# iit-DLSLab/gym-quadruped

Measured on AMD Instinct MI355X. Metric: env-steps/sec (batched), higher is better.
Workload: dtype f32; 1 GPU; mini_cheetah flat, 4096 envs/GPU, random-action rollout (50*N(0,1) torques), ALL_OBS (227 scalars), auto-reset on termination (next_step), sim_dt 0.002, newton solver <=100 it tol 1e-8, robot self-collision on (mesh pairs: GJK / EPA on the hulls, as mjc_Convex); envs_per_gpu=4096, total_envs=4096, parallelism=env-shards x1 (no collectives)

## Files before the change

### gym_quadruped_amd/csrc/gq_boxes.h

```cpp
#pragma once
#include "gq_step_kernel.h"
#include "gq_pairs.h"
#include "gq_convex.h"
#include "gq_exchange.h"

namespace gq {

#define GQ_BX_WCLS(W) (reinterpret_cast<int32_t*>(&(W).F[0][32]))
#define GQ_BX_LGNRM(W) (&(W).F[1][0])
#define GQ_BX_CONNRM(W) (&(W).F[1][3 * GQ_MAXLG])
#define GQ_BX_ISPH(W) (&(W).u.B[40][0])
#define GQ_BX_OBBW 13
#define GQ_BX_OBB(W) (&(W).u.B[0][0])
#define GQ_CVX_SHP(W) ((LdsF)&(W).F[0][44])
#define GQ_CVX_POLY_BOX(W) ((LdsF)&(W).u.B[28][0])
#define GQ_CVX_POLY_SELF(W) ((LdsF)&(W).u.B[38][0])
static_assert(GQ_BX_OBBW * GQ_MAXLG <= 28 * GQ_NVD && 28 * GQ_NVD + GQ_CVX_POLY_WORDS <= 40 * GQ_NVD && 38 * GQ_NVD + GQ_CVX_POLY_WORDS <= 64 * GQ_NVD && 44 + GQ_CVX_SHP_WORDS <= GQ_FACTOR_SIZE,
              "scratch of the convex routine");

__device__ __forceinline__ float sphere_box(V3 c, V3 s, float r, V3& n) {
  const V3 q = v3(med3(c.x, -s.x, s.x), med3(c.y, -s.y, s.y), med3(c.z, -s.z, s.z));
  const V3 d = c - q;
  const float l2 = dot(d, d);
  if (l2 > 0.0f) {
// ... 530 lines not shown
  } else {
    const int tot = bcast(wave_incl_scan(nfit | ((nfit * need) << 8) | ((nfit * vres) << 18)), 63);
    const int found = bcast(incl_all, 63) & 0xff;
    ncon += tot & 0xff;
    rows += (tot >> 8) & 0x3ff;
    if constexpr (CONE) reserve += (tot >> 18) & 0x3ff;
    S.ndrop += found - (tot & 0xff);
  }
}

__device__ __forceinline__ void closest_seg_seg(V3 p1, V3 q1, V3 p2, V3 q2, V3& c1, V3& c2) {
  const V3 d1 = q1 - p1, d2 = q2 - p2, r = p1 - p2;
  const float a = dot(d1, d1), e = dot(d2, d2), f = dot(d2, r), EPS = 1e-12f;
  float s, t;
  if (a <= EPS && e <= EPS) { s = 0.0f; t = 0.0f; }
  else if (a <= EPS) { s = 0.0f; t = med3(fdiv(f, e), 0.0f, 1.0f); }
  else {
    const float c = dot(d1, r);
    if (e <= EPS) { t = 0.0f; s = med3(fdiv(-c, a), 0.0f, 1.0f); }
    else {
      const float b = dot(d1, d2), den = a * e - b * b;
      s = den > 1e-6f * a * e ? med3(fdiv(b * f - c * e, den), 0.0f, 1.0f) : 0.0f;
      const float ie = fast_rcp(e), ia = fast_rcp(a);
      t = (b * s + f) * ie;
      if (t < 0.0f) { t = 0.0f; s = med3(-c * ia, 0.0f, 1.0f); }
      else if (t > 1.0f) { t = 1.0f; s = med3((b - c) * ia, 0.0f, 1.0f); }
    }
  }
  c1 = p1 + s * d1; c2 = p2 + t * d2;
}

#define GQ_CON_BODY2(x) ((x) & 0xff)
#define GQ_CON_BODY1(x) (((x) >> 8) - 1)
#define GQ_WCLS_SELF (-2)

struct SelfPrefetch { float caps[7], bsph[4]; int32_t body, it1[2], it2[2], bp[2]; };
__device__ __forceinline__ SelfPrefetch self_prefetch(const GQ_MODEL GqDevModel& m, const int nlg, const int nsp) {
  const int lane = lane_id();
  SelfPrefetch P;
  const int it = lane < 4 + nlg ? lane : 0;
#pragma unroll
  for (int i = 0; i < 7; i++) P.caps[i] = m.item_caps[it][i];
#pragma unroll
  for (int i = 0; i < 4; i++) P.bsph[i] = m.item_bsph[it][i];
  P.body = m.item_body[it];
#pragma unroll
  for (int h = 0; h < 2; h++) {
    const int p = h * GQ_WAVE + lane < nsp ? h * GQ_WAVE + lane : 0;
    P.it1[h] = m.sp[p].it1; P.it2[h] = m.sp[p].it2; P.bp[h] = m.sp[p].bp;
  }
  return P;
}

__device__ inline void self_item_shape(const WaveMem& W, const GQ_MODEL GqDevModel& m, const int it, const float* k, LdsF dst) {
  CvxShape S;
  const int pt = it < 4 ? 2 : m.lg[it - 4].ptype;
  if (pt == 2 || pt == 3) {
    S.kind = 2; S.adr = 0; S.num = 2; S.pm = -1; S.t = ld3(k); S.h = ld3(k + 3); S.r = k[6];
#pragma unroll
    for (int i = 0; i < 9; i++) S.R[i] = (i % 4 == 0) ? 1.0f : 0.0f;
  } else {
    const GQ_MODEL GqDevGeom& G = m.lg[it - 4];
    const float* Rb = W.xmat[G.body];
    S.kind = 0; S.adr = G.plane_adr; S.num = G.cloud_num; S.pm = G.cap_adr; S.r = G.radius; S.h = v3(0.0f, 0.0f, 0.0f);
#pragma unroll
    for (int i = 0; i < 3; i++)
#pragma unroll
      for (int j = 0; j < 3; j++) S.R[3 * i + j] = Rb[3 * i] * G.mat[j] + Rb[3 * i + 1] * G.mat[3 + j] + Rb[3 * i + 2] * G.mat[6 + j];
    S.t = ld3(W.xpos[G.body]) + matvec(Rb, ld3(G.pos));
  }
  cvx_shape_store(dst, S);
}
__device__ inline void self_item_obb(const WaveMem& W, const GQ_MODEL GqDevModel& m, const int it, const float* k, V3& c, float* R, V3& h) {
  const int pt = it < 4 ? 2 : m.lg[it - 4].ptype;
  if (pt == 2 || pt == 3) {
    const V3 p0 = ld3(k), p1 = ld3(k + 3);
    c = 0.5f * (p0 + p1);
    h = v3(0.5f * fabsf(p1.x - p0.x) + k[6], 0.5f * fabsf(p1.y - p0.y) + k[6], 0.5f * fabsf(p1.z - p0.z) + k[6]);
#pragma unroll
    for (int i = 0; i < 9; i++) R[i] = (i % 4 == 0) ? 1.0f : 0.0f;
  } else {
    const GQ_MODEL GqDevGeom& G = m.lg[it - 4];
    const float* Rb = W.xmat[G.body];
#pragma unroll
    for (int i = 0; i < 3; i++)
#pragma unroll
      for (int j = 0; j < 3; j++) R[3 * i + j] = Rb[3 * i] * G.mat[j] + Rb[3 * i + 1] * G.mat[3 + j] + Rb[3 * i + 2] * G.mat[6 + j];
    c = ld3(W.xpos[G.body]) + matvec(Rb, ld3(G.pos)) + matvec(R, ld3(G.aabb_c));
    h = v3(G.aabb_h[0] + G.radius, G.aabb_h[1] + G.radius, G.aabb_h[2] + G.radius);
  }
}

#define GQ_COLD_HINT(c) (COLD ? __builtin_expect((long)(c), 0L) : (long)(c))

__device__ inline void sepc_store(const WaveMem& W, float* row, V3 d) {
  const float dd = dot(d, d);
  V3 b = v3(0.0f, 0.0f, 0.0f);
  if (dd > 1e-24f) b = fast_rsqrt(dd) * matTvec(W.xmat[0], d);
  row[0] = b.x; row[1] = b.y; row[2] = b.z;
}

__device__ inline bool self_hulls_apart(const WaveMem& W, const GQ_MODEL GqDevModel& m, const GQ_MODEL float* vx, int it1, const float* k1, const float* R1,
                                        int it2, const float* k2, const float* R2, float marg, bool use_dir = false, V3 dir = {0.0f, 0.0f, 0.0f}) {
  V3 t[2]; float r[2]; int adr[2]; bool seg[2];
#pragma unroll
  for (int s = 0; s < 2; s++) {
    const int it = s ? it2 : it1; const float* k = s ? k2 : k1;
    const int pt = it < 4 ? 2 : m.lg[it - 4].ptype;
    seg[s] = pt == 2 || pt == 3;
    if (seg[s]) { t[s] = 0.5f * (ld3(k) + ld3(k + 3)); r[s] = k[6]; adr[s] = -1; }
    else { const GQ_MODEL GqDevGeom& G = m.lg[it - 4]; t[s] = ld3(W.xpos[G.body]) + matvec(W.xmat[G.body], ld3(G.pos)); r[s] = G.radius; adr[s] = G.hgrid_adr; if (adr[s] < 0) return false; }
  }
  const V3 d = use_dir ? dir : t[1] - t[0];
  const float dd = dot(d, d);
  if (!(dd > 1e-12f)) return false;
  const float hA = seg[0] ? fmaxf(dot(ld3(k1), d), dot(ld3(k1 + 3), d)) : dot(t[0], d) + cvx_hgrid(vx, adr[0], matTvec(R1, d));
  const float hB = seg[1] ? fmaxf(-dot(ld3(k2), d), -dot(ld3(k2 + 3), d)) : -dot(t[1], d) + cvx_hgrid(vx, adr[1], matTvec(R2, -1.0f * d));
  return -hA - hB > (marg + r[0] + r[1] + 1e-5f) * fast_sqrt(dd);
}

template <bool CONE, bool PRIM = true, bool COLD = false, bool CVX = true>
__device__ inline void append_self_contacts(WaveMem& W, const GQ_MODEL GqDevModel& m, float mu_env, WorldAppend& S, const SelfPrefetch& pre, const StepConsts& K, const int nlg, const GQ_MODEL GqDevBatch& Bt, float* xdbg = nullptr, const int env = 0) {
  constexpr int NP = PRIM ? 4 : 1;
  const int lane = lane_id();
  const int nsp = K.nsp;
  if (nsp == 0) return;
  int32_t* xq_tab = nullptr; int xq_slots = 0;
  float* sepc = nullptr;
  int xq_pre = 0;
  (void)Bt; (void)env; (void)xdbg;
  if constexpr (CVX) {
#ifndef GQ_XQ_OFF
    xq_tab = Bt.xq; xq_slots = Bt.xq_slots;
#endif
    sepc = Bt.sepc ? Bt.sepc + (size_t)env * Bt.sepc_stride : nullptr;
    if (xq_tab) { Xq X0; X0.q = xq_tab; X0.slots = xq_slots; xq_pre = ld_pub(xq_tab + xq_window(X0, wave_index()) + lane); }
  }
  const uint64_t lt = lane == 0 ? 0ull : (~0ull >> (64 - lane));
  float(*cw)[12] = reinterpret_cast<float(*)[12]>(&W.u.B[0][0]);
  {
    const int it = lane < 4 + nlg ? lane : 0;
    const int b = pre.body;
    const V3 o = ld3(W.xpos[b]);
    const V3 e0 = o + matvec(W.xmat[b], v3(pre.caps[0], pre.caps[1], pre.caps[2])), e1 = o + matvec(W.xmat[b], v3(pre.caps[3], pre.caps[4], pre.caps[5]));
    st3(cw[it], e0); st3(cw[it] + 3, e1);
    cw[it][6] = pre.caps[6];
    st3(cw[it] + 8, o + matvec(W.xmat[b], v3(pre.bsph[0], pre.bsph[1], pre.bsph[2])));
    cw[it][11] = pre.bsph[3];
  }
  uint64_t near[2] = {~0ull, ~0ull};
  if (nsp > 2 * GQ_WAVE) {
#pragma unroll
    for (int half = 0; half < 2; half++) {
      const int p = half * GQ_WAVE + lane;
      bool nr = false;
      if (p < m.nbp) {
        const GQ_MODEL GqDevBodyPair& P = m.bp[p];
        const V3 d = ld3(W.xpos[P.b2]) + matvec(W.xmat[P.b2], ld3(m.body_sph[P.b2])) - ld3(W.xpos[P.b1]) - matvec(W.xmat[P.b1], ld3(m.body_sph[P.b1]));
        const float rr = m.body_sph[P.b1][3] + m.body_sph[P.b2][3] + K.self_margin;
        nr = dot(d, d) < rr * rr;
      }
      near[half] = ballot(nr);
    }
  }
  uint64_t live_pass = ~0ull;
  if constexpr (CONE) if (nsp > 2 * GQ_WAVE) {
    const int np = (nsp + GQ_WAVE - 1) / GQ_WAVE, lp = lane < np ? lane : 0;
    const uint64_t pb0 = m.sp_pass_bp[lp][0], pb1 = m.sp_pass_bp[lp][1];
    live_pass = ballot(lane < np && ((near[0] & pb0) | (near[1] & pb1)) != 0);
  }
  if (K.self_cut == 1) { wave_barrier(); return; }
  wave_barrier();
  GQ_SUB(W, 1, 10);
  int32_t* list = reinterpret_cast<int32_t*>(&W.u.B[30][0]);
  int ncand = 0;
#pragma unroll 1
  for (int p0 = 0; p0 < nsp; p0 += GQ_WAVE) {
    if constexpr (CONE) if (!((live_pass >> (p0 / GQ_WAVE)) & 1ull)) continue;
    const int p = p0 + lane;
    bool cand;
    {
      int it1, it2, bp;
      if (p0 == 0) { it1 = pre.it1[0]; it2 = pre.it2[0]; bp = pre.bp[0]; }
      else if (p0 == GQ_WAVE) { it1 = pre.it1[1]; it2 = pre.it2[1]; bp = pre.bp[1]; }
      else { const GQ_MODEL GqDevSelfPair& P = m.sp[p < nsp ? p : 0]; it1 = P.it1; it2 = P.it2; bp = P.bp; }
      const bool nr = (near[(bp >> 6) & 1] >> (bp & 63)) & 1;
      const float* k1 = cw[it1] + 8;
      const float* k2 = cw[it2] + 8;
      const V3 dm = ld3(k2) - ld3(k1);
      const float reach = k1[3] + k2[3] + K.self_margin;
      cand = p < nsp && nr && dot(dm, dm) < reach * reach;
    }
    const uint64_t cm = ballot(cand);
    if (cm == 0) continue;
    const int at = ncand + popc64(cm & lt);
    if (cand && at < 2 * GQ_WAVE) list[at] = p;
    ncand += popc64(cm);
  }
  GQ_SUB(W, 1, 11);
  int xq_act = 0, xq_hlp = 0;
  if constexpr (CVX) { xq_act = bcast(xq_pre, 31); xq_hlp = bcast(xq_pre, 63); }
  if (K.self_cut == 2) return;
  if (ncand == 0) {
    if constexpr (!CVX) return;
    else {
      if (xq_tab == nullptr) return;
      Xq X0; X0.q = xq_tab; X0.slots = xq_slots;
      xq_mark_helper(X0, wave_index(), xq_hlp);
      if (!xq_is_hot(xq_act, wall_clock64())) return;
    }
  }
  if (ncand > 2 * GQ_WAVE) ncand = 2 * GQ_WAVE;
  wave_barrier();
  const int npass = ncand > 0 ? ncand : 1;
#pragma unroll 1
  for (int c0 = 0; c0 < npass; c0 += GQ_WAVE) {
    const bool cand = c0 + lane < ncand;
    const int p = cand ? list[c0 + lane] : 0;
    PairHit H;
    H.n = 0;
    int it1 = 0, it2 = 0;
    bool cvx = false;
    if (cand) {
      const GQ_MODEL GqDevSelfPair& Pp = m.sp[p];
      it1 = Pp.it1; it2 = Pp.it2;
      const int kind = Pp.kind;
      const float marg = Pp.mix.margin;
      const float* k1 = cw[it1];
      const float* k2 = cw[it2];
      if (kind == 0) {
        V3 c1, c2;
        closest_seg_seg(ld3(k1), ld3(k1 + 3), ld3(k2), ld3(k2 + 3), c1, c2);
        const V3 d = c2 - c1;
        const float l2 = dot(d, d), len = fast_sqrt(l2), dist = len - k1[6] - k2[6];
        if (dist < marg && len >= 1e-9f) {
          const V3 nrm = fast_rcp(len) * d;
          H.n = 1; H.dist[0] = dist; H.nrm[0] = nrm; H.pos[0] = c1 + (k1[6] + 0.5f * dist) * nrm;
        }
      } else if (kind == 4) { if constexpr (CVX) {
        V3 c1, h1, c2, h2; float R1[9], R2[9];
        self_item_obb(W, m, it1, k1, c1, R1, h1);
        self_item_obb(W, m, it2, k2, c2, R2, h2);
        cvx = !obb_apart(c1, R1, h1, c2, R2, h2, marg);
        if (cvx) cvx = !self_hulls_apart(W, m, K.vx, it1, k1, R1, it2, k2, R2, marg);
        if (cvx && sepc) {
          const float* c = sepc + 3 * Pp.cidx;
          const V3 dw = matvec(W.xmat[0], v3(c[0], c[1], c[2]));
          if (dot(dw, dw) > 0.25f) cvx = !self_hulls_apart(W, m, K.vx, it1, k1, R1, it2, k2, R2, marg, true, dw);
        }
      } } else if constexpr (PRIM) {
        const int ib = kind == 2 ? it2 : it1;
        bool continue_pair = true;
        const GQ_MODEL GqDevGeom& G = m.lg[ib - 4];
        const float* Rb = W.xmat[G.body];
        float A[9];
#pragma unroll
        for (int i = 0; i < 3; i++)
#pragma unroll
          for (int j = 0; j < 3; j++) A[3 * i + j] = Rb[3 * i] * G.mat[j] + Rb[3 * i + 1] * G.mat[3 + j] + Rb[3 * i + 2] * G.mat[6 + j];
        const V3 ca = ld3(W.xpos[G.body]) + matvec(Rb, ld3(G.pos)), ha = ld3(G.psize);
        if (kind == 3) {
          const GQ_MODEL GqDevGeom& G2 = m.lg[it2 - 4];
          {
            V3 nn;
            if (point_box(matTvec(A, ld3(k2 + 8) - ca), ha, nn) - k2[11] >= marg) continue_pair = false;
          }
          if (continue_pair) {
          const float* Rb2 = W.xmat[G2.body];
          float A2[9];
#pragma unroll
          for (int i = 0; i < 3; i++)
#pragma unroll
            for (int j = 0; j < 3; j++) A2[3 * i + j] = Rb2[3 * i] * G2.mat[j] + Rb2[3 * i + 1] * G2.mat[3 + j] + Rb2[3 * i + 2] * G2.mat[6 + j];
          box_box(ca, A, ha, ld3(W.xpos[G2.body]) + matvec(Rb2, ld3(G2.pos)), A2, ld3(G2.psize), marg, H);
          }
        } else {
          const float* kc = kind == 1 ? k2 : k1;
          capsule_box(ld3(kc), ld3(kc + 3), kc[6], ca, A, ha, marg, H);
          if (kind == 2) {
#pragma unroll
            for (int k = 0; k < 2; k++) H.nrm[k] = -1.0f * H.nrm[k];
          }
        }
      }
    }
    if constexpr (CVX) {
      uint64_t cm = ballot(cvx);
      if (K.self_cut == 5) cm = 0;
      if (K.self_cut == 6) cm &= cm - 1;
      Xq X; X.q = xq_tab; X.slots = xq_slots;
      uint64_t local = cm, own = 0;
      int myslot = -1;
      bool linger = X.q != nullptr && cm == 0 && c0 + GQ_WAVE >= npass && xq_is_hot(xq_act, wall_clock64());
      int t_ref = 0; bool t_set = false;
#define GQ_XSTAT(i, v) do { if (xdbg && lane == 0) xdbg[i] = (float)(v); } while (0)
#define GQ_XTIME(i) GQ_XSTAT(i, wall_clock64() & 0xFFFFF)
      int x_back = 0, x_help = 0; long long x_ticks = 0, x_t0 = 0; bool x_ld = false;
      if (cm) GQ_XSTAT(0, popc64(cm));
      if (X.q != nullptr && cm == 0 && ncand != 0 && c0 + GQ_WAVE >= npass) xq_mark_helper(X, wave_index(), xq_hlp);
      if (GQ_COLD_HINT(X.q != nullptr && (cm & (cm - 1)) != 0 && xq_is_hot(xq_hlp, wall_clock64()))) {
        const uint64_t rest = cm & (cm - 1);
        if ((rest >> lane) & 1ull) myslot = xq_reserve(X, wave_index(), opaque_lane(lane));
        own = ballot(myslot >= 0);
        local = cm & ~own;
        for (uint64_t r = own; r;) {
          const int jj = ffs64(r); r &= r - 1;
          const int pj = bcast(p, jj), i1 = bcast(it1, jj), i2 = bcast(it2, jj), sj = bcast(myslot, jj);
          wave_barrier();
          self_item_shape(W, m, i1, cw[i1], GQ_CVX_SHP(W));
          self_item_shape(W, m, i2, cw[i2], GQ_CVX_SHP(W) + GQ_CVX_SHAPE_WORDS);
          wave_barrier();
          xq_put(X, sj, GQ_CVX_SHP(W), m.sp[pj].mix.margin);
        }
        publish_fence();
        if (myslot >= 0) { xq_ready(X, myslot); xq_mark_active(X, myslot); }
        GQ_XSTAT(1, popc64(own)); GQ_XTIME(2);
      }
      if (GQ_COLD_HINT(local != 0 || own != 0 || linger))
#pragma unroll 1
      for (;;) {
        int j = -1, slot = -1;
        if (local) { j = ffs64(local); local &= local - 1; }
        else if (own) {
          if (xdbg && !x_ld) { GQ_XTIME(3); x_ld = true; }
          const int s = myslot >= 0 ? ld_pub(xq_state(X, myslot)) : XQ_DONE;
          const uint64_t ready = ballot(s == XQ_READY), busy = ballot(s == XQ_CLAIMED);
          if (ready) {
            j = ffs64(ready);
            slot = bcast(myslot, j);
            if (!xq_claim(X, slot)) continue;
            j = -1; x_back++;
          } else if (busy) {
            if (!t_set) { t_ref = (int)wall_clock64(); t_set = true; }
            if ((int)wall_clock64() - t_ref < GQ_XQ_OWNER_TICKS) { nap(); continue; }
            j = ffs64(busy);
            own &= ~(1ull << j);
            if (lane == j) myslot = -1;
          } else break;
        } else if (linger) {
          if (!t_set) { t_ref = (int)wall_clock64(); t_set = true; }
          slot = xq_scan(X, wave_index());
          if (slot >= 0) {
            if (!xq_claim(X, slot)) continue;
            if (xdbg) { if (x_help == 0) GQ_XTIME(7); x_help++; x_t0 = wall_clock64(); }
          } else {
            if ((int)wall_clock64() - t_ref > GQ_XQ_LINGER_TICKS) break;
            nap();
            continue;
          }
        } else break;
        float marg;
        wave_barrier();
        if (j >= 0) {
          const int pj = bcast(p, j), i1 = bcast(it1, j), i2 = bcast(it2, j);
          self_item_shape(W, m, i1, cw[i1], GQ_CVX_SHP(W));
          self_item_shape(W, m, i2, cw[i2], GQ_CVX_SHP(W) + GQ_CVX_SHAPE_WORDS);
          marg = m.sp[pj].mix.margin;
        } else xq_get(X, slot, GQ_CVX_SHP(W), marg);
        wave_barrier();
        const bool hit = cvx_pair_wave(GQ_CVX_SHP(W), GQ_CVX_POLY_SELF(W), K.vx, K.vy, K.vz, marg);
        LdsCF out = GQ_CVX_SHP(W) + 2 * GQ_CVX_SHAPE_WORDS;
        if (j >= 0) {
          if (hit && lane == j) { H.n = 1; H.dist[0] = out[0]; H.nrm[0] = ld3(out + 1); H.pos[0] = ld3(out + 4); }
          if (!hit && lane == j && sepc) sepc_store(W, sepc + 3 * m.sp[p].cidx, ld3(out + 1));
        } else {
          wave_barrier(); xq_done(X, slot, hit, out);
          if (xdbg && linger) x_ticks += wall_clock64() - x_t0;
          if (linger && (int)wall_clock64() - t_ref > GQ_XQ_LINGER_TICKS) linger = false;
        }
      }
      if (xdbg) { if (own) { GQ_XTIME(4); GQ_XSTAT(5, x_back); } if (x_help) { GQ_XSTAT(6, x_help); GQ_XSTAT(8, x_ticks); } if (cm == 0 && X.q) GQ_XTIME(9); }
      if (own) {
        if (myslot >= 0) {
          const int32_t* it = xq_item(X, myslot);
          if (ld_pub(it + GQ_XQ_RES) != 0) {
            const float* r = reinterpret_cast<const float*>(it) + GQ_XQ_RES;
            H.n = 1; H.dist[0] = ld_pub(r + 1); H.nrm[0] = v3(ld_pub(r + 2), ld_pub(r + 3), ld_pub(r + 4)); H.pos[0] = v3(ld_pub(r + 5), ld_pub(r + 6), ld_pub(r + 7));
          }
          else if (sepc) { const float* r = reinterpret_cast<const float*>(it) + GQ_XQ_RES; sepc_store(W, sepc + 3 * m.sp[p].cidx, v3(ld_pub(r + 2), ld_pub(r + 3), ld_pub(r + 4))); }
          st_pub(xq_state(X, myslot), XQ_FREE);
        }
      }
    }
    const int cnt = H.n;
    if (ballot(cnt > 0) == 0 || K.self_cut == 4) continue;
    const GQ_MODEL GqDevSelfPair& P = m.sp[cnt > 0 ? p : 0];
    const int dim = P.mix.dim;
    float mu = 0.0f;
    if (cnt > 0) {
      const float f1 = it1 < 4 ? (mu_env >= 0.0f ? mu_env : m.foot_friction[it1][0]) : m.lg[it1 - 4].friction[0];
      const float f2 = it2 < 4 ? (mu_env >= 0.0f ? mu_env : m.foot_friction[it2][0]) : m.lg[it2 - 4].friction[0];
      mu = fmaxf(1e-5f, P.mix.rule == 0 ? fmaxf(f1, f2) : (P.mix.rule == 1 ? f1 : f2));
    }
    int& ncon = S.ncon; int& rows = S.rows; int& reserve = S.reserve;
    const int need = dim == 1 ? 1 : (CONE ? dim : 2 * (dim - 1));
    const int vres = (CONE && need > 1) ? need - 1 : 0;
    int idx0, rows0, res0, incl_all = 0;
    if constexpr (NP == 1) {
      idx0 = ncon + popc64(ballot(cnt > 0) & lt);
      const bool kept = cnt > 0 && idx0 < GQ_MAXCON;
      const uint64_t m1 = ballot(kept && need == 1), m3 = ballot(kept && need == 3), m4 = ballot(kept && need == 4), m6 = ballot(kept && need == 6);
      rows0 = rows + popc64(m1 & lt) + 3 * popc64(m3 & lt) + 4 * popc64(m4 & lt) + 6 * popc64(m6 & lt);
      res0 = CONE ? reserve + 2 * popc64(m3 & lt) + 5 * popc64(m6 & lt) : 0;
    } else {
      const int packed = cnt | ((cnt * need) << 8) | ((cnt * vres) << 18);
      incl_all = wave_incl_scan(packed);
      const int excl = incl_all - packed;
      idx0 = ncon + (excl & 0xff); rows0 = rows + ((excl >> 8) & 0x3ff); res0 = reserve + ((excl >> 18) & 0x3ff);
    }
    int nfit = 0;
#pragma unroll
    for (int k = 0; k < NP; k++) {
      if (k < cnt) {
        const int idx = idx0 + k, row0 = rows0 + k * need, res = res0 + (k + 1) * vres;
        const bool fits = S.ndrop == 0 && idx < GQ_MAXCON && row0 + need + res <= (CONE ? 64 : GQ_MAXEFC) && row0 + need <= GQ_MAXEFC;
        if (fits) {
          const int b1 = m.item_body[it1], b2 = m.item_body[it2];
          W.con_geom[idx] = it2 | ((it1 + 1) << 8) | (P.mix.rule << 16); W.con_body[idx] = b2 | ((b1 + 1) << 8); W.con_dim[idx] = dim; W.con_row[idx] = row0;
          W.con_dist[idx] = H.dist[k]; W.con_inc[idx] = P.mix.includemargin; W.con_mu[idx] = mu;
          st3(W.con_pos[idx], H.pos[k]);
          W.con_solref[idx][0] = P.mix.solref[0]; W.con_solref[idx][1] = P.mix.solref[1];
#pragma unroll
          for (int q = 0; q < 5; q++) W.con_solimp[idx][q] = P.mix.solimp[q];
          st3(GQ_BX_CONNRM(W) + 3 * idx, hit_nrm(H, k));
          GQ_BX_WCLS(W)[idx] = GQ_WCLS_SELF;
#ifdef GQ_EMU_TRACE
          if (getenv("GQ_EMU_TRACE")) printf("self contact idx %d items %d %d kind %d point %d dist %.6f pos %.5f %.5f %.5f nrm %.5f %.5f %.5f\n", idx, it1, it2, (int)m.sp[p].kind, k, (double)H.dist[k], (double)H.pos[k].x, (double)H.pos[k].y, (double)H.pos[k].z, (double)hit_nrm(H, k).x, (double)hit_nrm(H, k).y, (double)hit_nrm(H, k).z);
#endif
          nfit++;
        }
      }
    }
    if constexpr (NP == 1) {
      const uint64_t f1 = ballot(nfit && need == 1), f3 = ballot(nfit && need == 3), f4 = ballot(nfit && need == 4), f6 = ballot(nfit && need == 6);
      ncon += popc64(f1 | f3 | f4 | f6);
      rows += popc64(f1) + 3 * popc64(f3) + 4 * popc64(f4) + 6 * popc64(f6);
      if constexpr (CONE) reserve += 2 * popc64(f3) + 5 * popc64(f6);
      S.nself += popc64(f1 | f3 | f4 | f6);
      S.ndrop += popc64(ballot(cnt > 0)) - popc64(f1 | f3 | f4 | f6);
    } else {
      const int tot = bcast(wave_incl_scan(nfit | ((nfit * need) << 8) | ((nfit * vres) << 18)), 63);
      const int found = bcast(incl_all, 63) & 0xff;
      ncon += tot & 0xff;
      rows += (tot >> 8) & 0x3ff;
      if constexpr (CONE) reserve += (tot >> 18) & 0x3ff;
      S.nself += tot & 0xff;
      S.ndrop += found - (tot & 0xff);
    }
  }
}

template <bool CONE, bool PRIM = true, bool CVX = true>
__device__ __forceinline__ void stage_self_contacts(WaveMem& W, const GQ_MODEL GqDevModel& m, float mu_env, const SelfPrefetch& pre, const StepConsts& K, const int nlg, const GQ_MODEL GqDevBatch& Bt, float* xdbg = nullptr, const int env = 0) {
  const int lane = lane_id();
  WorldAppend S;
  S.ncon = uniform(W.ncon); S.rows = uniform(W.nefc); S.invalid = 0; S.reserve = 0; S.nself = 0; S.ndrop = uniform(W.ndrop);
  const int ncon = S.ncon;
  {
    const int lc = lane < GQ_MAXCON ? lane : GQ_MAXCON - 1;
    st3(GQ_BX_CONNRM(W) + 3 * lc, v3(0.0f, 0.0f, 1.0f));
    GQ_BX_WCLS(W)[lc] = -1;
  }
  if constexpr (CONE)
    for (int c = 0; c < ncon; c++) { const int d = uniform(W.con_dim[c]); S.reserve += d > 1 ? d - 1 : 0; }
  append_self_contacts<CONE, PRIM, false, CVX>(W, m, mu_env, S, pre, K, nlg, Bt, xdbg, env);
  { W.ncon = S.ncon; W.nefc = S.rows; W.nself = S.nself; W.ndrop = S.ndrop; }
  wave_barrier();
}

template <bool CONE, bool SELF, bool PRIM>
__device__ __forceinline__ void stage_box_contacts(WaveMem& W, const GQ_MODEL GqDevModel& m, const GQ_MODEL float* vx, const GQ_MODEL float* vy, const GQ_MODEL float* vz,
                                          double bx, double by, float mu_env, const SelfPrefetch& pre, const ItemRegs& IT, const StepConsts& K, const int nlg, const GQ_MODEL GqDevBatch& Bt, float* xdbg = nullptr, const int env = 0) {
  const int lane = lane_id();
  const PrimLane PL = prim_lane(W, m, IT, PRIM && lane < 4 + m.nlg, PRIM);
  WorldAppend S;
  S.ncon = uniform(W.ncon); S.rows = uniform(W.nefc); S.invalid = uniform(W.invalid); S.reserve = 0; S.nself = 0; S.ndrop = uniform(W.ndrop);
  S.ft = uniform(W.foot_touch) & 15;
  const int ncon = S.ncon;
  {
    const int lc = lane < GQ_MAXCON ? lane : GQ_MAXCON - 1;
    st3(GQ_BX_CONNRM(W) + 3 * lc, v3(0.0f, 0.0f, 1.0f));
    GQ_BX_WCLS(W)[lc] = -1;
  }
  if constexpr (CONE)
    for (int c = 0; c < ncon; c++) { const int d = uniform(W.con_dim[c]); S.reserve += d > 1 ? d - 1 : 0; }
  uint64_t cand[2];
  {
    V3 cg; float rg;
    item_sphere(W, m, false, cg, rg);
    box_candidates(W, m, bx, by, 0.0f, cand, cg, rg);
    if (lane < GQ_MAXLG) { st3(GQ_BX_ISPH(W) + 4 * lane, cg); GQ_BX_ISPH(W)[4 * lane + 3] = rg; }
    item_obb_store(W, m);
  }
  wave_barrier();
#pragma unroll 1
  for (int half = 0; half < 2; half++) {
    uint64_t todo = cand[half];
    while (todo) {
      const int b = half * GQ_WAVE + ffs64(todo);
      todo &= todo - 1;
      PairHit H;
      const float* sph = GQ_BX_ISPH(W) + 4 * opaque_lane(lane < GQ_MAXLG ? lane : 0);
      const V3 cg = ld3(sph); const float rg = sph[3];
      if (!box_item_scan<PRIM, 1, true>(W, m, vx, vy, vz, b, bx, by, 0.0f, cg, rg, PL, H)) continue;
      append_world_contacts<CONE, PRIM>(W, m, m.box[b].cls, mu_env, H, S);
      wave_barrier();
    }
  }
  if (m.hf_nrow > 0) {
    float dist; V3 nrm, pt;
    const float* sph = GQ_BX_ISPH(W) + 4 * opaque_lane(lane < GQ_MAXLG ? lane : 0);
    const V3 cg = ld3(sph); const float rg = sph[3];
    if (hfield_item_scan(W, m, vx, vy, vz, bx, by, 0.0f, cg, rg, dist, nrm, pt)) {
      PairHit H;
      H.n = dist < 1e29f ? 1 : 0; H.dist[0] = dist; H.nrm[0] = nrm; H.pos[0] = pt;
      append_world_contacts<CONE, false>(W, m, m.hf_cls, mu_env, H, S);
      wave_barrier();
    }
// ... 15 lines not shown
```

### gym_quadruped_amd/csrc/gq_step_body.h

```cpp
#pragma once
#include "gq_step_kernel.h"
#include "gq_newton.h"
#include "gq_boxes.h"
#include "gq_heightmap.h"

namespace gq {

__device__ __forceinline__ float m_entry(const WaveMem& W, int i, int j) {
  if (i < j) { int t = i; i = j; j = t; }
  if (i < 6) return W.Mb[i][j];
  if (j < 6) return W.Mc[i - 6][j];
  if ((i - 6) / 3 != (j - 6) / 3) return 0.0f;
  return W.Mc[i - 6][6 + (j - 6) % 3];
}

__device__ inline Q4 stage_kinematics(WaveMem& W, const GqDevLinkRec L) {
  const int lane = lane_id();
  Q4 qbase = {W.qb[0], W.qb[1], W.qb[2], W.qb[3]};
  qbase = qnormalize(qbase);
  {
    W.xpos[0][0] = 0.0f; W.xpos[0][1] = 0.0f; W.xpos[0][2] = W.basez;
    q2mat(W.xmat[0], qbase);
  }
  {
// ... 527 lines not shown
    W.u.dyn.crb[b0 + 2][k] = c2; W.u.dyn.crb[b0 + 1][k] = c1; W.u.dyn.crb[b0][k] = c0;
  }
  wave_barrier();
  { const int l10 = lane < 10 ? lane : 9; W.u.dyn.crb[0][l10] = W.u.dyn.cinert[0][l10] + W.u.dyn.crb[1][l10] + W.u.dyn.crb[4][l10] + W.u.dyn.crb[7][l10] + W.u.dyn.crb[10][l10]; }
  wave_barrier();

  GQ_TICK(2); GQ_SUB(W, 1, 4);
  {
    static_assert(sizeof(WaveMem::Mc) == 108 * 4 && offsetof(WaveMem, Mb) == offsetof(WaveMem, Mc) + sizeof(WaveMem::Mc), "S3 writes Mc | Mb as one flat array");
    float* M0 = &W.Mc[0][0];
#pragma unroll
    for (int p = 0; p < 3; p++) {
      const int ent = s3e[p], dd = ent & 0xff, sa = (ent >> 8) & 0xff, bd = (ent >> 16) & 0xff;
      float buf[6];
      mul_inert(buf, W.u.dyn.crb[bd], W.cdof[dd]);
      const float* sv = W.cdof[sa];
      const float v = sv[0] * buf[0] + sv[1] * buf[1] + sv[2] * buf[2] + sv[3] * buf[3] + sv[4] * buf[4] + sv[5] * buf[5];
      const int e = lane + GQ_WAVE * p;
      M0[e < 143 ? e : 143] = (ent >> 24) ? v + s3a[p] : 0.0f;
    }
  }
  wave_barrier();

  GQ_TICK(3); GQ_SUB(W, 1, 5);
  if constexpr (SOLVER == 0 && !(BOXES || SELF)) factor_tree_both(W, m.dof_damping, h);

  GQ_TICK(4);
  const int nlg = C.nlg;
  const ItemRegs IT = item_fetch(m, lane < 4 + nlg ? lane : 0);
  const FootRec FRec = foot_fetch(m, lane);
  const int l12_ = lane < GQ_NJ ? lane : GQ_NJ - 1, l18_ = lane < GQ_NVD ? lane : GQ_NVD - 1;
  constexpr bool EARLY = !CONE && !(BOXES && PRIM);
#define GQ_FETCH_LIM() do { lim_on = m.lim_rec[l12_].limited; lim_lo_ = m.lim_rec[l12_].lo; lim_hi_ = m.lim_rec[l12_].hi; lim_mg = m.lim_rec[l12_].margin; } while (0)
#define GQ_FETCH_FLR() do { flr_dof = m.fl_row[l18_].dof; flr_R = m.fl_row[l18_].R; flr_B = m.fl_row[l18_].B; flr_floss = m.fl_row[l18_].floss; } while (0)
#define GQ_FETCH_HENT() do { if constexpr (SOLVER == 1) { hent_pre[0] = m.newton_hent[0][lane]; hent_pre[1] = m.newton_hent[1][lane]; } else { hent_pre[0] = hent_pre[1] = 0; } } while (0)
  int lim_on = 0, flr_dof = 0, hent_pre[2] = {0, 0};
  float lim_lo_ = 0.0f, lim_hi_ = 0.0f, lim_mg = 0.0f, flr_R = 0.0f, flr_B = 0.0f, flr_floss = 0.0f;
  if constexpr (EARLY) { GQ_FETCH_LIM(); GQ_FETCH_FLR(); GQ_FETCH_HENT(); }
  auto fetch_lim = [&]() { GQ_FETCH_LIM(); };
  auto fetch_flr = [&]() { GQ_FETCH_FLR(); };
  auto fetch_hent = [&]() { GQ_FETCH_HENT(); };
  StepConsts K;
  {
    int fl0 = m.hot_foot_leg[0], fl1 = m.hot_foot_leg[1], fl2 = m.hot_foot_leg[2], fl3 = m.hot_foot_leg[3], its = m.iterations, nsp = m.hot_nsp, scut = m.hot_self_cut;
    float fmu = m.hot_floor_mu, imr = m.impratio, gz = m.gravity_z, mi = m.meaninertia, tol = m.tolerance, nf = m.noise_floor, smg = m.hot_self_margin;
    const GQ_MODEL float* vxq = mptr(a.vx); const GQ_MODEL float* vyq = mptr(a.vy); const GQ_MODEL float* vzq = mptr(a.vz);
    pin(fl0); pin(fl1); pin(fl2); pin(fl3); pin(its); pin(nsp); pin(scut); pin(fmu); pin(imr); pin(gz); pin(mi); pin(tol); pin(nf); pin(smg);
    pin(vxq); pin(vyq); pin(vzq);
    K.foot_leg[0] = fl0; K.foot_leg[1] = fl1; K.foot_leg[2] = fl2; K.foot_leg[3] = fl3; K.iterations = its; K.nsp = nsp; K.self_cut = scut;
    K.floor_mu = fmu; K.impratio_rs = fast_rsqrt(imr); K.gravity_z = gz; K.nw_scale = fast_rcp(mi * 18.0f); K.tolerance = tol; K.noise_floor = nf; K.self_margin = smg;
    K.vx = vxq; K.vy = vyq; K.vz = vzq;
  }
  const GQ_MODEL float* vx_p = K.vx; const GQ_MODEL float* vy_p = K.vy; const GQ_MODEL float* vz_p = K.vz;
  {
    float vb[6], ab[6];
    {
      const float* R = W.xmat[0];
      V3 wl = v3(W.qvel[3], W.qvel[4], W.qvel[5]);
      V3 ww = matvec(R, wl), vl = v3(W.qvel[0], W.qvel[1], W.qvel[2]);
      st3(vb, ww); st3(vb + 3, vl);
      V3 al = cross(vl, ww);
      ab[0] = ab[1] = ab[2] = 0.0f; ab[3] = al.x; ab[4] = al.y; ab[5] = al.z - K.gravity_z;
#pragma unroll
      for (int k = 0; k < 6; k++) { W.u.dyn.cvel[0][k] = vb[k]; W.u.dyn.cacc[0][k] = ab[k]; }
    }
#pragma unroll
    for (int i = 0; i < 3; i++) {
      const int b = 1 + 3 * lq + i, d = 6 + 3 * lq + i;
      float cd[6];
      cross_motion(cd, vb, W.cdof[d]);
      float qd = W.qvel[d];
#pragma unroll
      for (int k = 0; k < 6; k++) { vb[k] += W.cdof[d][k] * qd; ab[k] += cd[k] * qd; W.u.dyn.cvel[b][k] = vb[k]; W.u.dyn.cacc[b][k] = ab[k]; }
    }
  }
  wave_barrier();
  {
    float t1[6], t2[6], f[6];
    mul_inert(t1, W.u.dyn.cinert[lb], W.u.dyn.cacc[lb]);
    mul_inert(t2, W.u.dyn.cinert[lb], W.u.dyn.cvel[lb]);
    cross_force(f, W.u.dyn.cvel[lb], t2);
#pragma unroll
    for (int k = 0; k < 6; k++) W.u.dyn.cfrc[lb][k] = f[k] + t1[k];
  }
  wave_barrier();
  {
    const int l24 = lane < 24 ? lane : 23;
    const int leg = l24 / 6, k = l24 % 6, b0 = 1 + 3 * leg;
    float f2 = W.u.dyn.cfrc[b0 + 2][k], f1 = W.u.dyn.cfrc[b0 + 1][k] + f2, f0 = W.u.dyn.cfrc[b0][k] + f1;
    wave_barrier();
    W.u.dyn.cfrc[b0 + 1][k] = f1; W.u.dyn.cfrc[b0][k] = f0;
  }
  wave_barrier();
  {
    const int l6 = lane < 6 ? lane : 5;
    const float fb = W.u.dyn.cfrc[0][l6] + (W.u.dyn.cfrc[1][l6] + W.u.dyn.cfrc[4][l6] + W.u.dyn.cfrc[7][l6] + W.u.dyn.cfrc[10][l6]);
    wave_barrier();
    W.u.dyn.cfrc[0][l6] = fb;
  }
  wave_barrier();
  {
    const float* s = W.cdof[ld];
    const float* f = W.u.dyn.cfrc[dof_body(ld)];
    float bias = s[0] * f[0] + s[1] * f[1] + s[2] * f[2] + s[3] * f[3] + s[4] * f[4] + s[5] * f[5];
    const float sm_new = W.smooth[ld] - bias;
    wave_barrier();
    W.bias[ld] = bias;
    W.smooth[ld] = sm_new;
  }

  GQ_TICK(5); GQ_SUB(W, 1, 6);
  SelfPrefetch self_pre;
  if constexpr (SELF && !BOXES) self_pre = self_prefetch(m, nlg, K.nsp);
  stage_collision_scan(W, m, vx_p, vy_p, vz_p, false, FRec);
  GQ_SUB(W, 1, 7);
  const int nitem = 4 + nlg;
  FloorCand FC;
  FC.n = 0; FC.r = 0.0f; FC.t1c = 0.0f; FC.t1s = 1.0f; FC.key = 0xE4;
#pragma unroll
  for (int k = 0; k < 4; k++) { FC.dist[k] = 1e30f; FC.pt[k] = v3(0.0f, 0.0f, 0.0f); }
  int code = 0, body = 0, dim = 3, fric_rule = 0;
  bool calf = false;
  float cmargin = 0.0f, inc = 0.0f, fgeom = 0.0f;
  float solref[2] = {0.02f, 1.0f}, solimp[5] = {0.9f, 0.95f, 0.001f, 0.5f, 2.0f};
  if (lane < nitem) {
    floor_candidates(W, IT, FC);
    code = IT.code; cmargin = IT.margin; body = IT.body; dim = IT.dim; inc = IT.inc; calf = IT.calf != 0;
    fgeom = IT.friction0; fric_rule = IT.fric_rule;
    solref[0] = IT.solref[0]; solref[1] = IT.solref[1];
#pragma unroll
    for (int q = 0; q < 5; q++) solimp[q] = IT.solimp[q];
  }
  if (uniform(GQ_LIFT_DUE(W))) {
    float dz = 0.0f;
    for (int it = 0; it < 100; it++) {
      float pen = 0.0f;
      bool touching = false;
#pragma unroll
      for (int k = 0; k < 4; k++) {
        const bool tk = calf && k < FC.n && FC.dist[k] + dz < cmargin;
        touching = touching || tk;
        pen = tk ? fmaxf(pen, fabsf(FC.dist[k] + dz)) : pen;
      }
      if (ballot(touching) == 0) break;
      dz += 1.1f * wave_max(pen);
    }
    bool still = false;
#pragma unroll
    for (int k = 0; k < 4; k++) still = still || (calf && k < FC.n && FC.dist[k] + dz < cmargin);
    const int failed = ballot(still) != 0;
    wave_barrier();
    if (lane == 0) { W.basez += dz; if (a.lift_failed) gptr(a.lift_failed)[env] = (uint8_t)failed; }
    if (lane < GQ_NB) W.xpos[lane][2] += dz;
    if (lane < 4) W.foot_world[lane][2] += dz;
#pragma unroll
    for (int k = 0; k < 4; k++) { FC.dist[k] += dz; FC.pt[k].z += dz; }
    wave_barrier();
  }
  GQ_TICK(14); GQ_SUB(W, 1, 8);
  if (a.dyn && rec_pass) {
    GQ_GLOBAL float* D = gptr(a.dyn) + (size_t)env * GQ_DYN_STRIDE;
    const float* Mc0 = &W.Mc[0][0];
    const float* Mb0 = &W.Mb[0][0];
    const float* xp0 = &W.xpos[0][0];
    const float* xm0 = &W.xmat[0][0];
    D[GQ_DYN_MC + lane] = Mc0[lane];
// ... 988 lines not shown
```

Before: 32.46 million env-steps/s.

## Publish previously-touching convex self pairs to the exchange queue before collision scan

Convex self-collision pairs that were in contact on the previous step are now marked in the separating-direction cache with a sentinel. Early in the step, before the floor collision scan, those pairs' shapes are published to the cross-wave exchange queue so helper waves can start GJK/EPA sooner. Later, append_self_contacts reuses the reserved slots and skips re-testing those pairs. This overlaps the expensive hull narrowphase with other stage work, at the cost of extra bookkeeping, LDS hand-over words and added barriers. It also risks publishing pairs that have since separated.

```diff
diff --git a/gym_quadruped_amd/csrc/gq_boxes.h b/gym_quadruped_amd/csrc/gq_boxes.h
--- a/gym_quadruped_amd/csrc/gq_boxes.h
+++ b/gym_quadruped_amd/csrc/gq_boxes.h
@@ -606,6 +606,18 @@
   return P;
 }
 
+#define GQ_SELF_END_POINTS(W, pre, nlg, lane, cw) \
+  {  \
+    const int it = lane < 4 + nlg ? lane : 0; \
+    const int b = pre.body; \
+    const V3 o = ld3(W.xpos[b]); \
+    const V3 e0 = o + matvec(W.xmat[b], v3(pre.caps[0], pre.caps[1], pre.caps[2])), e1 = o + matvec(W.xmat[b], v3(pre.caps[3], pre.caps[4], pre.caps[5])); \
+    st3(cw[it], e0); st3(cw[it] + 3, e1); \
+    cw[it][6] = pre.caps[6]; \
+    st3(cw[it] + 8, o + matvec(W.xmat[b], v3(pre.bsph[0], pre.bsph[1], pre.bsph[2])));  \
+    cw[it][11] = pre.bsph[3]; \
+  }
+
 __device__ inline void self_item_shape(const WaveMem& W, const GQ_MODEL GqDevModel& m, const int it, const float* k, LdsF dst) {
   CvxShape S;
   const int pt = it < 4 ? 2 : m.lg[it - 4].ptype;
@@ -654,6 +666,91 @@
   row[0] = b.x; row[1] = b.y; row[2] = b.z;
 }
 
+#define GQ_SEPC_TOUCH 2.0f
+__device__ __forceinline__ void sepc_touch(float* row) { row[0] = GQ_SEPC_TOUCH; row[1] = 0.0f; row[2] = 0.0f; }
+
+#define GQ_XQ_EARLY_MAX 32
+#define GQ_XE_MASK(W) (reinterpret_cast<uint32_t*>(&(W).force[2]))
+#define GQ_XE_SLOT(W) (reinterpret_cast<int32_t*>(&(W).force[8]))
+static_assert((8 + GQ_XQ_EARLY_MAX) * sizeof(float) <= sizeof(WaveMem::force), "hand-over words of the early publication: force[2 .. 8 + GQ_XQ_EARLY_MAX)");
+
+struct EarlyPrefetch { float s[2]; };
+__device__ __forceinline__ EarlyPrefetch early_prefetch(const GQ_MODEL GqDevBatch& Bt, const int env) {
+  const int lane = lane_id();
+  EarlyPrefetch E;
+  const int stride = Bt.sepc_stride;
+  const float* sepc = Bt.sepc ? Bt.sepc + (size_t)env * stride : nullptr;
+#pragma unroll
+  for (int h = 0; h < 2; h++) {
+    const int w = 3 * (h * GQ_WAVE + lane);
+    E.s[h] = (sepc && w < stride) ? sepc[w] : 0.0f;
+  }
+  return E;
+}
+
+__device__ __forceinline__ uint64_t low_bits(uint64_t x, int k) {
+  uint64_t r = 0;
+  for (; k > 0 && x; k--) { r |= x & (~x + 1); x &= x - 1; }
+  return r;
+}
+
+__device__ inline void early_publish(WaveMem& W, const GQ_MODEL GqDevModel& m, const SelfPrefetch& pre, const EarlyPrefetch& E, const StepConsts& K, const int nlg,
+                                     const GQ_MODEL GqDevBatch& Bt, float* xdbg, const bool cut) {
+  const int lane = lane_id();
+  const uint64_t rows[2] = {ballot(E.s[0] == GQ_SEPC_TOUCH), ballot(E.s[1] == GQ_SEPC_TOUCH)};
+  if (lane < 4) GQ_XE_MASK(W)[lane] = 0u;
+  if (xdbg && lane == 0) xdbg[10] = 0.0f;
+  if ((rows[0] | rows[1]) == 0) return;
+#ifdef GQ_XQ_OFF
+  return;
+#else
+  Xq X; X.q = Bt.xq; X.slots = Bt.xq_slots;
+  if (cut || X.q == nullptr || K.self_cut != 0 || uniform(GQ_LIFT_DUE(W)) != 0) return;
+  const int xq_pre = ld_pub(X.q + xq_window(X, wave_index()) + lane);
+  int cidx[2];
+#pragma unroll
+  for (int h = 0; h < 2; h++) cidx[h] = h * GQ_WAVE + lane < K.nsp ? m.sp[h * GQ_WAVE + lane].cidx : -1;
+  float(*cw)[12] = reinterpret_cast<float(*)[12]>(&W.u.B[0][0]);
+  GQ_SELF_END_POINTS(W, pre, nlg, lane, cw)
+  wave_barrier();
+  if (!xq_is_hot(bcast(xq_pre, 63), wall_clock64())) return;
+  uint64_t em[2];
+#pragma unroll
+  for (int h = 0; h < 2; h++) em[h] = ballot(cidx[h] >= 0 && cidx[h] < 2 * GQ_WAVE && (((cidx[h] < GQ_WAVE ? rows[0] : rows[1]) >> (cidx[h] & 63)) & 1ull) != 0);
+  em[0] = low_bits(em[0], GQ_XQ_EARLY_MAX);
+  em[1] = low_bits(em[1], GQ_XQ_EARLY_MAX - popc64(em[0]));
+  int myslot[2] = {-1, -1};
+#pragma unroll
+  for (int h = 0; h < 2; h++)
+    if ((em[h] >> lane) & 1ull) myslot[h] = xq_reserve(X, wave_index(), opaque_lane(lane) + h * GQ_WAVE);
+  uint64_t got[2];
+#pragma unroll
+  for (int h = 0; h < 2; h++) {
+    got[h] = ballot(myslot[h] >= 0);
+    for (uint64_t r = got[h]; r;) {
+      const int jj = ffs64(r); r &= r - 1;
+      const int i1 = bcast(pre.it1[h], jj), i2 = bcast(pre.it2[h], jj), sj = bcast(myslot[h], jj);
+      wave_barrier();
+      self_item_shape(W, m, i1, cw[i1], GQ_CVX_SHP(W));
+      self_item_shape(W, m, i2, cw[i2], GQ_CVX_SHP(W) + GQ_CVX_SHAPE_WORDS);
+      wave_barrier();
+      xq_put(X, sj, GQ_CVX_SHP(W), m.sp[h * GQ_WAVE + jj].mix.margin);
+    }
+  }
+  publish_fence();
+  const uint64_t lt = lane == 0 ? 0ull : (~0ull >> (64 - lane));
+#pragma unroll
+  for (int h = 0; h < 2; h++)
+    if (myslot[h] >= 0) {
+      xq_ready(X, myslot[h]); xq_mark_active(X, myslot[h]);
+      GQ_XE_SLOT(W)[(h ? popc64(got[0]) : 0) + popc64(got[h] & lt)] = myslot[h];
+    }
+  if (lane < 4) GQ_XE_MASK(W)[lane] = (uint32_t)(((lane & 2) ? got[1] : got[0]) >> (32 * (lane & 1)));
+  if (xdbg && lane == 0) { xdbg[10] = (float)(popc64(got[0]) + popc64(got[1])); xdbg[11] = (float)(wall_clock64() & 0xFFFFF); }
+  wave_barrier();
+#endif
+}
+
 __device__ inline bool self_hulls_apart(const WaveMem& W, const GQ_MODEL GqDevModel& m, const GQ_MODEL float* vx, int it1, const float* k1, const float* R1,
                                         int it2, const float* k2, const float* R2, float marg, bool use_dir = false, V3 dir = {0.0f, 0.0f, 0.0f}) {
   V3 t[2]; float r[2]; int adr[2]; bool seg[2];
@@ -673,7 +770,7 @@
   return -hA - hB > (marg + r[0] + r[1] + 1e-5f) * fast_sqrt(dd);
 }
 
-template <bool CONE, bool PRIM = true, bool COLD = false, bool CVX = true>
+template <bool CONE, bool PRIM = true, bool COLD = false, bool CVX = true, bool XEARLY = false>
 __device__ inline void append_self_contacts(WaveMem& W, const GQ_MODEL GqDevModel& m, float mu_env, WorldAppend& S, const SelfPrefetch& pre, const StepConsts& K, const int nlg, const GQ_MODEL GqDevBatch& Bt, float* xdbg = nullptr, const int env = 0) {
   constexpr int NP = PRIM ? 4 : 1;
   const int lane = lane_id();
@@ -682,6 +779,7 @@
   int32_t* xq_tab = nullptr; int xq_slots = 0;
   float* sepc = nullptr;
   int xq_pre = 0;
+  uint64_t xe[2] = {0ull, 0ull};
   (void)Bt; (void)env; (void)xdbg;
   if constexpr (CVX) {
 #ifndef GQ_XQ_OFF
@@ -689,19 +787,15 @@
 #endif
     sepc = Bt.sepc ? Bt.sepc + (size_t)env * Bt.sepc_stride : nullptr;
     if (xq_tab) { Xq X0; X0.q = xq_tab; X0.slots = xq_slots; xq_pre = ld_pub(xq_tab + xq_window(X0, wave_index()) + lane); }
+    if constexpr (XEARLY) {
+      const uint32_t* e = GQ_XE_MASK(W);
+      xe[0] = (uint64_t)(uint32_t)uniform((int)e[0]) | ((uint64_t)(uint32_t)uniform((int)e[1]) << 32);
+      xe[1] = (uint64_t)(uint32_t)uniform((int)e[2]) | ((uint64_t)(uint32_t)uniform((int)e[3]) << 32);
+    }
   }
   const uint64_t lt = lane == 0 ? 0ull : (~0ull >> (64 - lane));
   float(*cw)[12] = reinterpret_cast<float(*)[12]>(&W.u.B[0][0]);
-  {
-    const int it = lane < 4 + nlg ? lane : 0;
-    const int b = pre.body;
-    const V3 o = ld3(W.xpos[b]);
-    const V3 e0 = o + matvec(W.xmat[b], v3(pre.caps[0], pre.caps[1], pre.caps[2])), e1 = o + matvec(W.xmat[b], v3(pre.caps[3], pre.caps[4], pre.caps[5]));
-    st3(cw[it], e0); st3(cw[it] + 3, e1);
-    cw[it][6] = pre.caps[6];
-    st3(cw[it] + 8, o + matvec(W.xmat[b], v3(pre.bsph[0], pre.bsph[1], pre.bsph[2])));
-    cw[it][11] = pre.bsph[3];
-  }
+  GQ_SELF_END_POINTS(W, pre, nlg, lane, cw)
   uint64_t near[2] = {~0ull, ~0ull};
   if (nsp > 2 * GQ_WAVE) {
 #pragma unroll
@@ -730,7 +824,9 @@
   int ncand = 0;
 #pragma unroll 1
   for (int p0 = 0; p0 < nsp; p0 += GQ_WAVE) {
-    if constexpr (CONE) if (!((live_pass >> (p0 / GQ_WAVE)) & 1ull)) continue;
+    uint64_t xep = 0ull;
+    if constexpr (XEARLY) xep = p0 == 0 ? xe[0] : (p0 == GQ_WAVE ? xe[1] : 0ull);
+    if constexpr (CONE) if (!((live_pass >> (p0 / GQ_WAVE)) & 1ull) && (!XEARLY || xep == 0)) continue;
     const int p = p0 + lane;
     bool cand;
     {
@@ -743,7 +839,8 @@
       const float* k2 = cw[it2] + 8;
       const V3 dm = ld3(k2) - ld3(k1);
       const float reach = k1[3] + k2[3] + K.self_margin;
-      cand = p < nsp && nr && dot(dm, dm) < reach * reach;
+      if constexpr (XEARLY) cand = p < nsp && ((nr && dot(dm, dm) < reach * reach) || ((xep >> lane) & 1ull));
+      else cand = p < nsp && nr && dot(dm, dm) < reach * reach;
     }
     const uint64_t cm = ballot(cand);
     if (cm == 0) continue;
@@ -775,6 +872,8 @@
     H.n = 0;
     int it1 = 0, it2 = 0;
     bool cvx = false;
+    bool pre_out = false;
+    if constexpr (CVX && XEARLY) pre_out = cand && p < 2 * GQ_WAVE && (((p < GQ_WAVE ? xe[0] : xe[1]) >> (p & 63)) & 1ull) != 0;
     if (cand) {
       const GQ_MODEL GqDevSelfPair& Pp = m.sp[p];
       it1 = Pp.it1; it2 = Pp.it2;
@@ -782,7 +881,8 @@
       const float marg = Pp.mix.margin;
       const float* k1 = cw[it1];
       const float* k2 = cw[it2];
-      if (kind == 0) {
+      if (XEARLY && pre_out) {
+      } else if (kind == 0) {
         V3 c1, c2;
         closest_seg_seg(ld3(k1), ld3(k1 + 3), ld3(k2), ld3(k2 + 3), c1, c2);
         const V3 d = c2 - c1;
@@ -800,7 +900,8 @@
         if (cvx && sepc) {
           const float* c = sepc + 3 * Pp.cidx;
           const V3 dw = matvec(W.xmat[0], v3(c[0], c[1], c[2]));
-          if (dot(dw, dw) > 0.25f) cvx = !self_hulls_apart(W, m, K.vx, it1, k1, R1, it2, k2, R2, marg, true, dw);
+          const float dd = dot(dw, dw);
+          if (dd > 0.25f && (!XEARLY || dd < 2.0f)) cvx =  !self_hulls_apart(W, m, K.vx, it1, k1, R1, it2, k2, R2, marg, true, dw);
         }
       } } else if constexpr (PRIM) {
         const int ib = kind == 2 ? it2 : it1;
@@ -843,21 +944,24 @@
       if (K.self_cut == 5) cm = 0;
       if (K.self_cut == 6) cm &= cm - 1;
       Xq X; X.q = xq_tab; X.slots = xq_slots;
-      uint64_t local = cm, own = 0;
+      const uint64_t xem = XEARLY ? ballot(pre_out) : 0ull;
+      uint64_t local = cm, own = xem;
       int myslot = -1;
-      bool linger = X.q != nullptr && cm == 0 && c0 + GQ_WAVE >= npass && xq_is_hot(xq_act, wall_clock64());
+      if (pre_out) myslot = GQ_XE_SLOT(W)[p < GQ_WAVE ? popc64(xe[0] & ((1ull << p) - 1ull)) : popc64(xe[0]) + popc64(xe[1] & ((1ull << (p - GQ_WAVE)) - 1ull))];
+      bool linger = X.q != nullptr && cm == 0 && xem == 0 && c0 + GQ_WAVE >= npass && xq_is_hot(xq_act, wall_clock64());
       int t_ref = 0; bool t_set = false;
 #define GQ_XSTAT(i, v) do { if (xdbg && lane == 0) xdbg[i] = (float)(v); } while (0)
 #define GQ_XTIME(i) GQ_XSTAT(i, wall_clock64() & 0xFFFFF)
       int x_back = 0, x_help = 0; long long x_ticks = 0, x_t0 = 0; bool x_ld = false;
-      if (cm) GQ_XSTAT(0, popc64(cm));
-      if (X.q != nullptr && cm == 0 && ncand != 0 && c0 + GQ_WAVE >= npass) xq_mark_helper(X, wave_index(), xq_hlp);
+      if (cm | xem) GQ_XSTAT(0, popc64(cm) + popc64(xem));
+      if (X.q != nullptr && cm == 0 && xem == 0 && ncand != 0 && c0 + GQ_WAVE >= npass) xq_mark_helper(X, wave_index(), xq_hlp);
       if (GQ_COLD_HINT(X.q != nullptr && (cm & (cm - 1)) != 0 && xq_is_hot(xq_hlp, wall_clock64()))) {
         const uint64_t rest = cm & (cm - 1);
         if ((rest >> lane) & 1ull) myslot = xq_reserve(X, wave_index(), opaque_lane(lane));
         own = ballot(myslot >= 0);
+        const uint64_t fresh = own & ~xem;
         local = cm & ~own;
-        for (uint64_t r = own; r;) {
+        for (uint64_t r = fresh; r;) {
           const int jj = ffs64(r); r &= r - 1;
           const int pj = bcast(p, jj), i1 = bcast(it1, jj), i2 = bcast(it2, jj), sj = bcast(myslot, jj);
           wave_barrier();
@@ -867,8 +971,8 @@
           xq_put(X, sj, GQ_CVX_SHP(W), m.sp[pj].mix.margin);
         }
         publish_fence();
-        if (myslot >= 0) { xq_ready(X, myslot); xq_mark_active(X, myslot); }
-        GQ_XSTAT(1, popc64(own)); GQ_XTIME(2);
+        if ((fresh >> lane) & 1ull) { xq_ready(X, myslot); xq_mark_active(X, myslot); }
+        GQ_XSTAT(1, popc64(fresh)); GQ_XTIME(2);
       }
       if (GQ_COLD_HINT(local != 0 || own != 0 || linger))
 #pragma unroll 1
@@ -915,7 +1019,7 @@
         const bool hit = cvx_pair_wave(GQ_CVX_SHP(W), GQ_CVX_POLY_SELF(W), K.vx, K.vy, K.vz, marg);
         LdsCF out = GQ_CVX_SHP(W) + 2 * GQ_CVX_SHAPE_WORDS;
         if (j >= 0) {
-          if (hit && lane == j) { H.n = 1; H.dist[0] = out[0]; H.nrm[0] = ld3(out + 1); H.pos[0] = ld3(out + 4); }
+          if (hit && lane == j) { H.n = 1; H.dist[0] = out[0]; H.nrm[0] = ld3(out + 1); H.pos[0] = ld3(out + 4); if (XEARLY && sepc) sepc_touch(sepc + 3 * m.sp[p].cidx); }
           if (!hit && lane == j && sepc) sepc_store(W, sepc + 3 * m.sp[p].cidx, ld3(out + 1));
         } else {
           wave_barrier(); xq_done(X, slot, hit, out);
@@ -930,6 +1034,7 @@
           if (ld_pub(it + GQ_XQ_RES) != 0) {
             const float* r = reinterpret_cast<const float*>(it) + GQ_XQ_RES;
             H.n = 1; H.dist[0] = ld_pub(r + 1); H.nrm[0] = v3(ld_pub(r + 2), ld_pub(r + 3), ld_pub(r + 4)); H.pos[0] = v3(ld_pub(r + 5), ld_pub(r + 6), ld_pub(r + 7));
+            if (XEARLY && sepc) sepc_touch(sepc + 3 * m.sp[p].cidx);
           }
           else if (sepc) { const float* r = reinterpret_cast<const float*>(it) + GQ_XQ_RES; sepc_store(W, sepc + 3 * m.sp[p].cidx, v3(ld_pub(r + 2), ld_pub(r + 3), ld_pub(r + 4))); }
           st_pub(xq_state(X, myslot), XQ_FREE);
@@ -1017,7 +1122,7 @@
   }
   if constexpr (CONE)
     for (int c = 0; c < ncon; c++) { const int d = uniform(W.con_dim[c]); S.reserve += d > 1 ? d - 1 : 0; }
-  append_self_contacts<CONE, PRIM, false, CVX>(W, m, mu_env, S, pre, K, nlg, Bt, xdbg, env);
+  append_self_contacts<CONE, PRIM, false, CVX, CVX>(W, m, mu_env, S, pre, K, nlg, Bt, xdbg, env);
   { W.ncon = S.ncon; W.nefc = S.rows; W.nself = S.nself; W.ndrop = S.ndrop; }
   wave_barrier();
 }
diff --git a/gym_quadruped_amd/csrc/gq_step_body.h b/gym_quadruped_amd/csrc/gq_step_body.h
--- a/gym_quadruped_amd/csrc/gq_step_body.h
+++ b/gym_quadruped_amd/csrc/gq_step_body.h
@@ -603,6 +603,9 @@
     K.vx = vxq; K.vy = vyq; K.vz = vzq;
   }
   const GQ_MODEL float* vx_p = K.vx; const GQ_MODEL float* vy_p = K.vy; const GQ_MODEL float* vz_p = K.vz;
+  EarlyPrefetch early_pre;
+  early_pre.s[0] = early_pre.s[1] = 0.0f;
+  if constexpr (SELF && !BOXES && CVX) early_pre = early_prefetch(Bt, env);
   {
     float vb[6], ab[6];
     {
@@ -663,6 +666,7 @@
   GQ_TICK(5); GQ_SUB(W, 1, 6);
   SelfPrefetch self_pre;
   if constexpr (SELF && !BOXES) self_pre = self_prefetch(m, nlg, K.nsp);
+  if constexpr (SELF && !BOXES && CVX) early_publish(W, m, self_pre, early_pre, K, nlg, Bt, (DBG && timing) ? call.debug + (size_t)env * GQ_DBG_SIZE + GQ_DBG_XQ : nullptr, MODE == 2 && call.stop_stage != 0);
   stage_collision_scan(W, m, vx_p, vy_p, vz_p, false, FRec);
   GQ_SUB(W, 1, 7);
   const int nitem = 4 + nlg;
```

Result: faster. 34.62 million env-steps/s, median of 6 (+6.7%).
